# kaiidams/Kokoro-Align

Hardware: AMD Instinct MI355X
Metric: aligned audio-frames/sec (whole node), 50k x 5k lattice (higher is better)
Workload: dtype f32; 1 GPU; cfg2: T=50000 x V=64 log-probs, S=5000 phonemes (L=10001), beam_size=1000, max_move=4; batch of 8192 independent lattices per GPU per step, as 4 launches of 2048 on 4 streams; lattices_per_gpu=8192, parallelism=lattice-sharded x1, kernel_form=auto, backtrace=auto, streams_per_gpu=4

## Files before the change

### kokoro-align_amd/csrc/ka_device.hpp

```cpp
#pragma once
#include "ka_types.hpp"

namespace ka {

__device__ __forceinline__ float ninf() { return -__builtin_inff(); }

__device__ __forceinline__ float wave_ror1(float x)
{
    return __builtin_bit_cast(float, __builtin_amdgcn_mov_dpp(__builtin_bit_cast(int, x), 0x13C, 0xF, 0xF, false));
}
__device__ __forceinline__ uint32_t shl1_in(uint32_t w, uint64_t mask)
{
    uint32_t r;
    uint64_t carry_out;
    asm("v_addc_co_u32 %0, %1, %2, %2, %3" : "=v"(r), "=&s"(carry_out) : "v"(w), "s"(mask));
    return r;
}
__device__ __forceinline__ float select_by_mask(float a, float b, uint64_t mask)
{
    float r;
    asm("v_cndmask_b32 %0, %1, %2, %3" : "=v"(r) : "v"(a), "v"(b), "s"(mask));
    return r;
}
__device__ __forceinline__ float bperm(int byte_addr, float src)
{
    return __builtin_bit_cast(float, __builtin_amdgcn_ds_bpermute(byte_addr, __builtin_bit_cast(int, src)));
}
__device__ __forceinline__ float first_lane(float x)
{
    return __builtin_bit_cast(float, __builtin_amdgcn_readfirstlane(__builtin_bit_cast(int, x)));
}

__device__ __forceinline__ float row_load(uint32_t lane_byte_off, const void *row_base )
{
    float r;
    asm volatile("global_load_dword %0, %1, %2" : "=v"(r) : "v"(lane_byte_off), "s"(row_base) : "memory");
    return r;
}
__device__ __forceinline__ void row_reload(float &r, uint32_t lane_byte_off, const void *row_base )
{
    asm volatile("global_load_dword %0, %1, %2" : "+v"(r) : "v"(lane_byte_off), "s"(row_base) : "memory");
}
typedef uint32_t u32x4 __attribute__((ext_vector_type(4)));
__device__ __forceinline__ u32x4 lp_descriptor(const void *base, uint64_t bytes)
{
    const uint64_t a = reinterpret_cast<uint64_t>(base);
    const uint32_t n = bytes > 0xffffffffull ? 0xffffffffu : (uint32_t)bytes;
    return u32x4{(uint32_t)__builtin_amdgcn_readfirstlane((int)(uint32_t)a), (uint32_t)__builtin_amdgcn_readfirstlane((int)((uint32_t)(a >> 32) & 0xffffu)),
                 (uint32_t)__builtin_amdgcn_readfirstlane((int)n), 0x00020000u};
}
__device__ __forceinline__ void row_reload_buf(float &r, uint32_t lane_byte_off, u32x4 rsrc , uint32_t row_byte_off )
{
    asm volatile("buffer_load_dword %0, %1, %2, %3 offen" : "+v"(r) : "v"(lane_byte_off), "s"(rsrc), "s"(row_byte_off) : "memory");
}
template <int N>
__device__ __forceinline__ void row_wait(float &r)
{
    asm volatile("s_waitcnt vmcnt(%1)" : "+v"(r) : "i"(N) : "memory");
}

__device__ __forceinline__ void row_wait_n(float &r, int n)
{
    switch (n) {
    case 0: row_wait<0>(r); break;
    case 1: row_wait<1>(r); break;
    case 2: row_wait<2>(r); break;
    case 3: row_wait<3>(r); break;
    case 4: row_wait<4>(r); break;
    case 5: row_wait<5>(r); break;
    case 6: row_wait<6>(r); break;
    case 7: row_wait<7>(r); break;
    case 8: row_wait<8>(r); break;
    case 9: row_wait<9>(r); break;
    case 10: row_wait<10>(r); break;
    case 11: row_wait<11>(r); break;
    case 12: row_wait<12>(r); break;
    case 13: row_wait<13>(r); break;
    case 14: row_wait<14>(r); break;
    case 15: row_wait<15>(r); break;
    case 16: row_wait<16>(r); break;
    case 17: row_wait<17>(r); break;
    case 18: row_wait<18>(r); break;
    case 19: row_wait<19>(r); break;
    case 20: row_wait<20>(r); break;
    case 21: row_wait<21>(r); break;
    case 22: row_wait<22>(r); break;
    case 23: row_wait<23>(r); break;
    case 24: row_wait<24>(r); break;
    case 25: row_wait<25>(r); break;
    case 26: row_wait<26>(r); break;
    case 27: row_wait<27>(r); break;
    case 28: row_wait<28>(r); break;
    case 29: row_wait<29>(r); break;
    case 30: row_wait<30>(r); break;
    case 31: row_wait<31>(r); break;
    default: row_wait<0>(r); break;
    }
}

struct BandMasks {
    uint64_t m0, m1, m2, m3, m4, m5, m6, m7, m8, m9, m10, m11, m12, m13, m14, m15;
    template <int K>
    __device__ __forceinline__ uint64_t &at()
    {
        if constexpr (K == 0) return m0;
        else if constexpr (K == 1) return m1;
        else if constexpr (K == 2) return m2;
        else if constexpr (K == 3) return m3;
        else if constexpr (K == 4) return m4;
        else if constexpr (K == 5) return m5;
        else if constexpr (K == 6) return m6;
        else if constexpr (K == 7) return m7;
        else if constexpr (K == 8) return m8;
        else if constexpr (K == 9) return m9;
        else if constexpr (K == 10) return m10;
        else if constexpr (K == 11) return m11;
        else if constexpr (K == 12) return m12;
        else if constexpr (K == 13) return m13;
        else if constexpr (K == 14) return m14;
        else return m15;
    }
};
template <int K>
__device__ __forceinline__ void band_rebuild_one(BandMasks &mk, uint32_t lo, uint32_t hi)
{
    const uint32_t first = (lo + 15u - (uint32_t)K) >> 4;
    const uint32_t last = (hi + 15u - (uint32_t)K) >> 4;
    const uint32_t cnt = last - first;
    const uint64_t m = cnt >= 64u ? ~0ull : ((1ull << cnt) - 1ull);
    const uint32_t r = first & 63u;
    mk.at<K>() = r ? ((m << r) | (m >> (64u - r))) : m;
    if constexpr (K < 15) band_rebuild_one<K + 1>(mk, lo, hi);
}
__device__ __forceinline__ void band_rebuild(BandMasks &mk, uint32_t lo, uint32_t hi) { band_rebuild_one<0>(mk, lo, hi); }
__device__ __forceinline__ void band_toggle(BandMasks &mk, uint32_t p)
{
    const uint64_t bit = 1ull << ((p >> 4) & 63u);
    const uint32_t k = p & 15u;
    asm volatile(
        "s_bitcmp1_b32 %16, 3\n\t"
        "s_cbranch_scc1 .Lka_8_16_%=\n\t"
        "s_bitcmp1_b32 %16, 2\n\t"
        "s_cbranch_scc1 .Lka_4_8_%=\n\t"
        "s_bitcmp1_b32 %16, 1\n\t"
        "s_cbranch_scc1 .Lka_2_4_%=\n\t"
        "s_bitcmp1_b32 %16, 0\n\t"
        "s_cbranch_scc1 .Lka_1_2_%=\n\t"
        "s_xor_b64 %0, %0, %17\n\t"
        "s_branch .Lka_end_%=\n\t"
        ".Lka_1_2_%=:\n\t"
        "s_xor_b64 %1, %1, %17\n\t"
        "s_branch .Lka_end_%=\n\t"
        ".Lka_2_4_%=:\n\t"
        "s_bitcmp1_b32 %16, 0\n\t"
        "s_cbranch_scc1 .Lka_3_2_%=\n\t"
        "s_xor_b64 %2, %2, %17\n\t"
        "s_branch .Lka_end_%=\n\t"
        ".Lka_3_2_%=:\n\t"
        "s_xor_b64 %3, %3, %17\n\t"
        "s_branch .Lka_end_%=\n\t"
        ".Lka_4_8_%=:\n\t"
        "s_bitcmp1_b32 %16, 1\n\t"
        "s_cbranch_scc1 .Lka_6_4_%=\n\t"
        "s_bitcmp1_b32 %16, 0\n\t"
        "s_cbranch_scc1 .Lka_5_2_%=\n\t"
        "s_xor_b64 %4, %4, %17\n\t"
        "s_branch .Lka_end_%=\n\t"
        ".Lka_5_2_%=:\n\t"
        "s_xor_b64 %5, %5, %17\n\t"
        "s_branch .Lka_end_%=\n\t"
        ".Lka_6_4_%=:\n\t"
        "s_bitcmp1_b32 %16, 0\n\t"
        "s_cbranch_scc1 .Lka_7_2_%=\n\t"
        "s_xor_b64 %6, %6, %17\n\t"
        "s_branch .Lka_end_%=\n\t"
        ".Lka_7_2_%=:\n\t"
        "s_xor_b64 %7, %7, %17\n\t"
        "s_branch .Lka_end_%=\n\t"
        ".Lka_8_16_%=:\n\t"
        "s_bitcmp1_b32 %16, 2\n\t"
        "s_cbranch_scc1 .Lka_12_8_%=\n\t"
        "s_bitcmp1_b32 %16, 1\n\t"
        "s_cbranch_scc1 .Lka_10_4_%=\n\t"
        "s_bitcmp1_b32 %16, 0\n\t"
        "s_cbranch_scc1 .Lka_9_2_%=\n\t"
        "s_xor_b64 %8, %8, %17\n\t"
        "s_branch .Lka_end_%=\n\t"
        ".Lka_9_2_%=:\n\t"
        "s_xor_b64 %9, %9, %17\n\t"
        "s_branch .Lka_end_%=\n\t"
        ".Lka_10_4_%=:\n\t"
        "s_bitcmp1_b32 %16, 0\n\t"
        "s_cbranch_scc1 .Lka_11_2_%=\n\t"
        "s_xor_b64 %10, %10, %17\n\t"
        "s_branch .Lka_end_%=\n\t"
        ".Lka_11_2_%=:\n\t"
        "s_xor_b64 %11, %11, %17\n\t"
        "s_branch .Lka_end_%=\n\t"
        ".Lka_12_8_%=:\n\t"
        "s_bitcmp1_b32 %16, 1\n\t"
        "s_cbranch_scc1 .Lka_14_4_%=\n\t"
        "s_bitcmp1_b32 %16, 0\n\t"
        "s_cbranch_scc1 .Lka_13_2_%=\n\t"
        "s_xor_b64 %12, %12, %17\n\t"
        "s_branch .Lka_end_%=\n\t"
        ".Lka_13_2_%=:\n\t"
        "s_xor_b64 %13, %13, %17\n\t"
        "s_branch .Lka_end_%=\n\t"
        ".Lka_14_4_%=:\n\t"
        "s_bitcmp1_b32 %16, 0\n\t"
        "s_cbranch_scc1 .Lka_15_2_%=\n\t"
        "s_xor_b64 %14, %14, %17\n\t"
        "s_branch .Lka_end_%=\n\t"
        ".Lka_15_2_%=:\n\t"
        "s_xor_b64 %15, %15, %17\n\t"
        "s_branch .Lka_end_%=\n\t"
        ".Lka_end_%=:\n\t"
        : "+s"(mk.m0), "+s"(mk.m1), "+s"(mk.m2), "+s"(mk.m3), "+s"(mk.m4), "+s"(mk.m5), "+s"(mk.m6), "+s"(mk.m7),
          "+s"(mk.m8), "+s"(mk.m9), "+s"(mk.m10), "+s"(mk.m11), "+s"(mk.m12), "+s"(mk.m13), "+s"(mk.m14), "+s"(mk.m15)
        : "s"(k), "s"(bit)
        : "scc");
}
__device__ __forceinline__ uint32_t pair_mask(int n)
{
    n = n < 0 ? 0 : n;
    return n >= 16 ? 0x55555555u : (((1u << (2 * n)) - 1u) & 0x55555555u);
}
__device__ __forceinline__ uint32_t band_pairs(uint32_t lo, uint32_t hi, int blk)
{
    const int p0 = blk * 16;
    return pair_mask((int)hi - p0) & ~pair_mask((int)lo - p0);
}
__device__ __forceinline__ void load_block_labels(gci32_t labx, int blk, int (&la)[8])
{
    gci4_t p = (gci4_t)(labx + (size_t)blk * 8);
    const v4i_t a = p[0], b = p[1];
    la[0] = a.x; la[1] = a.y; la[2] = a.z; la[3] = a.w;
    la[4] = b.x; la[5] = b.y; la[6] = b.z; la[7] = b.w;
}

__device__ __forceinline__ uint64_t feq(float a, float b) { return __builtin_amdgcn_fcmpf(a, b, 1 ); }

template <int M>
__device__ __forceinline__ void cell_blank(float a0, float a1, float a3, float e, float &m, uint32_t &word)
{
    const float c0 = a0 + e;
    if constexpr (M == 1) {
        m = c0;
        word = (word << 2) | 3u;
    } else {
        const float c1 = a1 + e;
        if constexpr (M <= 3) {
            m = __builtin_fmaxf(c0, c1);
            word = (shl1_in(word, feq(c0, m)) << 1) | 1u;
        } else {
            const float c3 = a3 + e;
            m = __builtin_fmaxf(__builtin_fmaxf(c0, c1), c3);
            word = shl1_in(shl1_in(word, feq(c0, m)), feq(c1, m));
        }
    }
}
template <int M, bool ZL>
__device__ __forceinline__ void cell_label(float a0, float a1, float a2, float a3, float e, float veto,
                                           float &m, uint32_t &word)
{
    const float c0 = a0 + e;
    if constexpr (M == 1) {
        m = c0;
        word = (word << 2) | 3u;
    } else {
        const float c1 = a1 + e;
        if constexpr (M == 2) {
            m = __builtin_fmaxf(c0, c1);
            const uint64_t e0 = feq(c0, m);
            word = shl1_in((word << 1) | 1u, e0);
        } else {
            float c2 = a2 + e;
            if constexpr (ZL) c2 = __builtin_fminf(c2, veto);
            if constexpr (M == 3) {
                m = __builtin_fmaxf(__builtin_fmaxf(c0, c1), c2);
                const uint64_t e0 = feq(c0, m), e1 = feq(c1, m);
                word = shl1_in(shl1_in(word, e0 | e1), ~e1 | e0);
            } else {
                const float c3 = a3 + e;
                m = __builtin_fmaxf(__builtin_fmaxf(__builtin_fmaxf(c0, c1), c2), c3);
                const uint64_t e0 = feq(c0, m), e1 = feq(c1, m), e2 = feq(c2, m);
                word = shl1_in(shl1_in(word, e0 | e1), e0 | (e2 & ~e1));
            }
        }
    }
}
__device__ __forceinline__ uint32_t blank_to_uniform(uint32_t x)
{
    const uint32_t h = (x >> 1) & 0x11111111u, l = x & 0x11111111u;
    return (x & 0xCCCCCCCCu) | ((h | l) << 1) | h;
}
__device__ __forceinline__ int bp_decode(uint32_t code) { return (int)(3u & ~code); }
__device__ __forceinline__ uint32_t live_pairs(uint32_t live2, uint32_t word, uint32_t band2)
{
    const uint32_t stay = (word >> 1) & (word | 0x11111111u);
    return (live2 | ~stay) & band2;
}

template <int M>
__device__ __forceinline__ float cell_blank_max(float a0, float a1, float a3)
{
    if constexpr (M == 1) return a0;
    if constexpr (M <= 3) return __builtin_fmaxf(a0, a1);
    return __builtin_fmaxf(__builtin_fmaxf(a0, a1), a3);
}
template <int M, bool ZL>
__device__ __forceinline__ float cell_label_max(float a0, float a1, float a2, float a3, float veto)
{
    if constexpr (M == 1) return a0;
    if constexpr (M == 2) return __builtin_fmaxf(a0, a1);
    if constexpr (ZL) a2 = __builtin_fminf(a2, veto);
    if constexpr (M == 3) return __builtin_fmaxf(__builtin_fmaxf(a0, a1), a2);
    return __builtin_fmaxf(__builtin_fmaxf(__builtin_fmaxf(a0, a1), a2), a3);
}
template <int M, bool ZL>
__device__ __forceinline__ f32x2 label_pair_max(float l1, float b1, float l0, float b0, float p1, float p2, float veto1, float veto0)
{
    if constexpr (M == 4 && !ZL) {
        const float m0 = __builtin_fmaxf(l0, b0);
        return f32x2{__builtin_fmaxf(__builtin_fmaxf(m0, p1), p2), __builtin_fmaxf(__builtin_fmaxf(l1, b1), m0)};
    } else {
        return f32x2{cell_label_max<M, ZL>(l0, b0, p1, p2, veto0), cell_label_max<M, ZL>(l1, b1, l0, b0, veto1)};
    }
}
#define KA_P(P, k) (P)[2 * ((k) >> 2) + ((k) & 1)][((k) >> 1) & 1]
__device__ __forceinline__ float lds_col(const float *row, int byte_addr)
{
    return *reinterpret_cast<const float *>(reinterpret_cast<const char *>(row) + byte_addr);
}
template <int M, bool ZL, int G>
__device__ __forceinline__ void frame_scores(f32x2 (&P)[8], float h1, float h2, float h3, f32x2 (&E)[4], const float (&vz)[8],
                                             f32x2 e00, const int (&la)[8], const float *next_row)
{
    const float b0 = P[2 * G][0], l0 = P[2 * G + 1][0], b1 = P[2 * G][1], l1 = P[2 * G + 1][1];
    const float p1 = G > 0 ? P[2 * (G > 0 ? G - 1 : 0) + 1][1] : h1;
    const float p2 = G > 0 ? P[2 * (G > 0 ? G - 1 : 0)][1] : h2;
    const float p3 = G > 0 ? P[2 * (G > 0 ? G - 1 : 0) + 1][0] : h3;
    f32x2 ml, mb;
    ml = label_pair_max<M, ZL>(l1, b1, l0, b0, p1, p2, vz[2 * G + 1], vz[2 * G]);
    mb[1] = cell_blank_max<M>(b1, l0, p1);
    mb[0] = cell_blank_max<M>(b0, p1, p3);
    P[2 * G + 1] = ml + E[G];
    P[2 * G] = mb + e00;
    E[G][0] = lds_col(next_row, la[2 * G]);
    E[G][1] = lds_col(next_row, la[2 * G + 1]);
    if constexpr (G > 0) frame_scores<M, ZL, G - 1>(P, h1, h2, h3, E, vz, e00, la, next_row);
}

template <int K>
__device__ __forceinline__ void mask_scores(f32x2 (&P)[8], BandMasks &mk, float NINF)
{
    KA_P(P, K) = select_by_mask(NINF, KA_P(P, K), mk.at<K>());
    if constexpr (K > 0) mask_scores<K - 1>(P, mk, NINF);
}

template <int M, bool ZL, int K>
__device__ __forceinline__ void frame_cells(float (&sc)[16], float h1, float h2, float h3, float (&ec)[8],
                                            const float (&vz)[8], float e0, BandMasks &mk, float NINF, uint32_t &word,
                                            const int (&la)[8], float next_row)
{
    const float a0 = sc[K];
    const float a1 = K >= 1 ? sc[K >= 1 ? K - 1 : 0] : h1;
    const float a2 = K >= 2 ? sc[K >= 2 ? K - 2 : 0] : (K == 1 ? h1 : h2);
    const float a3 = K >= 3 ? sc[K >= 3 ? K - 3 : 0] : (K == 2 ? h1 : (K == 1 ? h2 : h3));
    float m;
    if constexpr (K & 1) {
        cell_label<M, ZL>(a0, a1, a2, a3, ec[K >> 1], vz[K >> 1], m, word);
        ec[K >> 1] = bperm(la[K >> 1], next_row);
    } else {
        cell_blank<M>(a0, a1, a3, e0, m, word);
    }
    sc[K] = select_by_mask(NINF, m, mk.at<K>());
    if constexpr (K % 4 == 0) __builtin_amdgcn_sched_barrier(0);
    if constexpr (K > 0) frame_cells<M, ZL, K - 1>(sc, h1, h2, h3, ec, vz, e0, mk, NINF, word, la, next_row);
}



__device__ __forceinline__ int lattice_of_chunk(const Lattice *__restrict__ lats, int n, int64_t g)
{
    int lo = 0, hi = n - 1;
    while (lo < hi) {
        const int mid = (lo + hi + 1) >> 1;
        if (lats[mid].chunk0 <= g) lo = mid; else hi = mid - 1;
    }
    return lo;
}
__device__ __forceinline__ int chunks_of(int T) { return (T - 1) / kCkFrames + 1; }

__device__ __forceinline__ float wave_shr1(float first, float x)
{
    return __builtin_bit_cast(float, __builtin_amdgcn_update_dpp(__builtin_bit_cast(int, first), __builtin_bit_cast(int, x), 0x138, 0xF, 0xF, false));
}

__device__ __forceinline__ uint32_t cu_slot()
{
    uint32_t hw, xcc;
    asm volatile("s_getreg_b32 %0, hwreg(HW_REG_HW_ID)" : "=s"(hw));
    asm volatile("s_getreg_b32 %0, hwreg(HW_REG_XCC_ID)" : "=s"(xcc));
    return ((xcc & 7u) << 8) | ((hw >> 8) & 0xffu);
}

}
```

### kokoro-align_amd/csrc/ka_wave_forward.hpp

```cpp
#pragma once
#include "ka_device.hpp"

namespace ka {

__global__ __launch_bounds__(256) void prep_labels_kernel(const Lattice *__restrict__ lats, int32_t *meta)
{
    const Lattice &d = lats[blockIdx.x];
    int bad = 0, zero = 0;
    for (int i = threadIdx.x; i < d.labx_len; i += blockDim.x) {
        int v = 0;
        if (i < d.S) {
            int l = d.labels[i];
            if (l < 0 || l >= d.V) { bad = 1; l = 0; }
            if (l == 0) zero = 1;
            v = l * 4;
        }
        d.labx[i] = v;
    }
    int32_t *m = meta_of(meta, d.idx);
    if (bad) atomicMin(&m[0], kStatusBadLabel);
    if (zero) atomicOr(&m[2], 1);
}

template <int M, bool ZL>
__device__ __forceinline__ void forward_w16(const Lattice &d, int32_t *meta)
{
    constexpr int D = kRowDepth;
    const int lane = threadIdx.x;
    const uint32_t T = (uint32_t)__builtin_amdgcn_readfirstlane(d.T);
    const uint32_t L = (uint32_t)__builtin_amdgcn_readfirstlane(d.L);
    const uint32_t B = (uint32_t)__builtin_amdgcn_readfirstlane(d.beam);
    const uint32_t halfB = B >> 1;
    const uint32_t dq = L / T, dr = L % T;
    const float NINF = ninf();

    float sc[16];
#pragma unroll
    for (int k = 0; k < 16; ++k) sc[k] = NINF;
    if (lane == 0) sc[0] = 0.0f;
    uint32_t pres2 = lane == 0 ? 1u : 0u;
    bool pend_reset = false;
    bool reset_lane = false;

    int blk = lane;
    uint32_t blo = 0;
    int la[8];
    float vz[8];
    gci32_t labx = (gci32_t)d.labx;
    load_block_labels(labx, blk, la);
#pragma unroll
    for (int i = 0; i < 8; ++i) vz[i] = (ZL && la[i] == 0) ? NINF : __builtin_inff();

    uint32_t q = 0, rem = 0;
    uint32_t lo = 0, hi = B < L ? B : L;
    BandMasks mk;
    band_rebuild(mk, lo, hi);
    uint32_t band2 = band_pairs(lo, hi, blk);

    const uint32_t lane_off = (lane < d.V ? (uint32_t)lane : 0u) * 4u;
    const char *lp = reinterpret_cast<const char *>(d.lp);
    const size_t ld = (size_t)d.ld * 4;
    float rows[D];
#pragma unroll
    for (int i = 0; i < D; ++i) {
        const uint32_t tt = (uint32_t)i < T ? (uint32_t)i : T - 1;
        rows[i] = row_load(lane_off, lp + (size_t)tt * ld);
    }
#pragma unroll
    for (int i = 0; i < D; ++i) row_wait<0>(rows[i]);
    float e[8], e0[2];
#pragma unroll
    for (int i = 0; i < 8; ++i) e[i] = bperm(la[i], rows[0]);
    e0[0] = first_lane(rows[0]);
    float absum = __builtin_fabsf(rows[0]);

    const uint32_t *bp = reinterpret_cast<const uint32_t *>(d.bp);
    const uint32_t lane_store_off = (uint32_t)lane * 16u;

    const char *row_ahead = lp + (size_t)(D < T ? D : T - 1) * ld;
    uint32_t step_thr = dq != 0 ? 0u : T;
    asm("" : "+s"(step_thr));
    for (uint32_t tb = 0; tb < T; tb += D) {
        uint32_t gw[4];
#pragma unroll
        for (int i = 0; i < 4; ++i) asm("" : "=v"(gw[i]));
#pragma unroll
        for (int dd = 0; dd < D; ++dd) {
            const uint32_t t = tb + dd;
            if (t < T) {
                float h1 = wave_ror1(sc[15]), h2 = wave_ror1(sc[14]), h3 = wave_ror1(sc[13]);
                if (__builtin_expect(pend_reset, 0)) {
                    asm volatile("" ::: "memory");
                    const bool left_reset = __builtin_amdgcn_update_dpp(0, (int)reset_lane, 0x13C, 0xF, 0xF, false) != 0;
                    const bool kill = reset_lane && left_reset;
                    h1 = kill ? NINF : h1;
                    h2 = kill ? NINF : h2;
                    h3 = kill ? NINF : h3;
#pragma unroll
                    for (int k = 0; k < 16; ++k) sc[k] = reset_lane ? NINF : sc[k];
                    pres2 = reset_lane ? 0u : pres2;
                    pend_reset = false;
                }
                bool moved = false;
                rem += dr;
                if (__builtin_expect(rem >= step_thr, 0)) {
                    asm volatile("" ::: "memory");
                    q += dq;
                    if (rem >= T) { rem -= T; ++q; }
                    if (t + 1 != T) {
                        moved = true;
                        const int32_t dlo = (int32_t)q - (int32_t)halfB;
                        const uint32_t nlo = (uint32_t)(dlo > 0 ? dlo : 0);
                        if ((nlo >> 4) != blo) {
                            blo = nlo >> 4;
                            const int nb = (int)blo + ((lane - (int)blo) & 63);
                            reset_lane = nb != blk;
                            if (nb != blk) {
                                blk = nb;
                                load_block_labels(labx, blk, la);
#pragma unroll
                                for (int i = 0; i < 8; ++i) asm volatile("" : "+v"(la[i]));
                            }
                            pend_reset = true;
                        }
                    }
                }
                if (dd < D - 1) row_wait<D - 1>(rows[(dd + 1) % D]); else row_wait<D - 2>(rows[(dd + 1) % D]);
                const float rn = rows[(dd + 1) % D];
                e0[(dd + 1) & 1] = first_lane(rn);
                absum += __builtin_fabsf(rn);
                uint32_t word = 0;
                frame_cells<M, ZL, 15>(sc, h1, h2, h3, e, vz, e0[dd & 1], mk, NINF, word, la, rn);
                gw[dd] = word;
                pres2 = live_pairs(pres2, word, band2);
                row_reload(rows[dd], lane_off, row_ahead);
                row_ahead += t + D + 1 < T ? ld : 0;
                if (moved) {
                    const int32_t dlo = (int32_t)q - (int32_t)halfB;
                    const uint32_t nlo = (uint32_t)(dlo > 0 ? dlo : 0);
                    const uint32_t nhi = (L - nlo < B) ? L : nlo + B;
                    if (nlo != lo || nhi != hi) {
                        if (nhi - hi <= 1u && nlo - lo <= 1u) {
                            if (nhi != hi) band_toggle(mk, hi);
                            if (nlo != lo) band_toggle(mk, lo);
                        } else {
                            band_rebuild(mk, nlo, nhi);
                        }
                        band2 = band_pairs(nlo, nhi, blk);
                        lo = nlo;
                        hi = nhi;
                        if (ZL && pend_reset) {
#pragma unroll
                            for (int i = 0; i < 8; ++i) vz[i] = la[i] == 0 ? NINF : __builtin_inff();
                        }
                    }
                }
            }
        }
        const u32x4 words = {gw[0], gw[1], gw[2], gw[3]};
        asm volatile("global_store_dwordx4 %0, %1, %2\n\ts_nop 1" : : "v"(lane_store_off), "v"(words), "s"(bp + (size_t)tb * 64) : "memory");
    }

#pragma unroll
    for (int i = 0; i < D; ++i) row_wait<0>(rows[i]);

    int32_t *m = meta_of(meta, d.idx);
    if (__builtin_amdgcn_ballot_w64((__builtin_bit_cast(uint32_t, absum) & 0x7fffffffu) > 0x7f800000u)) {
        if (lane == 0) {
            m[1] = -1;
            atomicMin(&m[0], kStatusNaN);
        }
        return;
    }
    int best = -1;
    if (pres2) best = blk * 16 + ((31 - __clz((int)pres2)) >> 1);
#pragma unroll
    for (int off = 32; off >= 1; off >>= 1) {
        const int o = __shfl_xor(best, off);
        best = o > best ? o : best;
    }
    if (best < 0) {
        if (lane == 0) {
            m[1] = -1;
            atomicMin(&m[0], kStatusEmptyBeam);
        }
    } else if ((best >> 4) == blk) {
        float v = sc[0];
#pragma unroll
        for (int k = 1; k < 16; ++k) v = (best & 15) == k ? sc[k] : v;
        m[1] = best;
        m[3] = __builtin_bit_cast(int32_t, v);
    }
}

template <int M, bool ZL>
__device__ __forceinline__ void forward_ck(const Lattice &d, int32_t *meta)
{
    constexpr int D = kRowDepth;
    const int lane = threadIdx.x;
    const uint32_t T = (uint32_t)__builtin_amdgcn_readfirstlane(d.T);
    const uint32_t L = (uint32_t)__builtin_amdgcn_readfirstlane(d.L);
    const uint32_t B = (uint32_t)__builtin_amdgcn_readfirstlane(d.beam);
    const uint32_t halfB = B >> 1;
    const uint32_t dq = L / T, dr = L % T;
    const float NINF = ninf();

    f32x2 P[8];
#pragma unroll
    for (int k = 0; k < 16; ++k) KA_P(P, k) = NINF;
    if (lane == 0) KA_P(P, 0) = 0.0f;
    float absum = 0.0f;

    int blk = lane;
    uint32_t blo = 0;
    int la[8];
    float vz[8];
    gci32_t labx = (gci32_t)d.labx;
    load_block_labels(labx, blk, la);
#pragma unroll
    for (int i = 0; i < 8; ++i) vz[i] = (ZL && la[i] == 0) ? NINF : __builtin_inff();

    uint32_t q = 0, rem = 0;
    uint32_t lo = 0, hi = B < L ? B : L;
    BandMasks mk;
    band_rebuild(mk, lo, hi);

    const uint32_t lane_off = (lane < d.V ? (uint32_t)lane : 0u) * 4u;
    const char *lp = reinterpret_cast<const char *>(d.lp);
    const size_t ld = (size_t)d.ld * 4;
    float rows[D];
#pragma unroll
    for (int i = 0; i < D; ++i) {
        const uint32_t tt = (uint32_t)i < T ? (uint32_t)i : T - 1;
        rows[i] = row_load(lane_off, lp + (size_t)tt * ld);
    }
#pragma unroll
    for (int i = 0; i < D; ++i) row_wait<0>(rows[i]);
    f32x2 E[4];
    float e0[2];
    __shared__ float lrow[64];
    lrow[lane] = rows[0];
#pragma unroll
    for (int i = 0; i < 8; ++i) E[i >> 1][i & 1] = lds_col(lrow, la[i]);
    e0[0] = first_lane(rows[0]);
    absum = __builtin_fabsf(rows[0]);

    const char *ckp = reinterpret_cast<const char *>(d.bp);
    const uint32_t ld32 = (uint32_t)__builtin_amdgcn_readfirstlane((int)(uint32_t)ld), last_row = (T - 1u) * ld32;
    uint32_t row_ahead = (D < T ? (uint32_t)D : T - 1u) * ld32;
    const u32x4 lp_rsrc = lp_descriptor(d.lp, (uint64_t)T * ld);
    const uint32_t thr_real = dq != 0 ? 0u : T;
    const uint32_t mask_every4 = 1024u - (B < L ? B : L) >= 8u * (M - 1) ? 0u : 4u;
    uint32_t thr = thr_real;
    asm("" : "+s"(thr));
    float h1 = wave_ror1(KA_P(P, 15)), h2 = wave_ror1(KA_P(P, 14)), h3 = wave_ror1(KA_P(P, 13));
    for (uint32_t tb = 0; tb < T; tb += D) {
#pragma unroll
        for (int dd = 0; dd < D; ++dd) {
            const uint32_t t = tb + dd;
            if (t < T) {
                row_wait<D - 2>(rows[(dd + 1) % D]);
                const float rn = rows[(dd + 1) % D];
                lrow[lane] = rn;
                e0[(dd + 1) & 1] = first_lane(rn);
                absum += __builtin_fabsf(rn);
                const float e0t = e0[dd & 1];
                frame_scores<M, ZL, 3>(P, h1, h2, h3, E, vz, f32x2{e0t, e0t}, la, lrow);
                row_reload_buf(rows[dd], lane_off, lp_rsrc, row_ahead);
                row_ahead = min(row_ahead + ld32, last_row);
                if (dd == D - 1 && ((tb | mask_every4) & 4u) != 0) {
                    mask_scores<15>(P, mk, NINF);
                    if (((tb + D) & (kCkFrames - 1)) == 0 && tb + D < T) {
                        const char *ck = ckp + ((size_t)((tb + D) / kCkFrames) - 1) * 4096;
#pragma unroll
                        for (int g = 0; g < 4; ++g) {
                            const f32x4 v = {KA_P(P, 4 * g), KA_P(P, 4 * g + 1), KA_P(P, 4 * g + 2), KA_P(P, 4 * g + 3)};
                            asm volatile("global_store_dwordx4 %0, %1, %2 offset:%3\n\ts_nop 1" : : "v"((uint32_t)lane * 64u), "v"(v), "s"(ck), "i"(16 * g) : "memory");
                        }
                    }
                }
                h1 = wave_ror1(KA_P(P, 15));
                h2 = wave_ror1(KA_P(P, 14));
                h3 = wave_ror1(KA_P(P, 13));
                rem += dr;
                if (__builtin_expect(rem >= thr, 0)) {
                    asm volatile("" ::: "memory");
                    thr = thr_real;
                    if (dd != D - 1 || ((tb | mask_every4) & 4u) == 0) {
                        mask_scores<15>(P, mk, NINF);
                        h1 = wave_ror1(KA_P(P, 15));
                        h2 = wave_ror1(KA_P(P, 14));
                        h3 = wave_ror1(KA_P(P, 13));
                    }
                    if (rem >= thr_real) {
                        q += dq;
                        if (rem >= T) { rem -= T; ++q; }
                        if (t + 1 != T) {
                            const int32_t dlo = (int32_t)q - (int32_t)halfB;
                            const uint32_t nlo = (uint32_t)(dlo > 0 ? dlo : 0);
                            const uint32_t nhi = (L - nlo < B) ? L : nlo + B;
                            if ((nlo >> 4) != blo) {
                                blo = nlo >> 4;
                                const int nb = (int)blo + ((lane - (int)blo) & 63);
                                const bool reset_lane = nb != blk;
                                if (reset_lane) {
                                    blk = nb;
                                    load_block_labels(labx, blk, la);
#pragma unroll
                                    for (int i = 0; i < 8; ++i) asm volatile("" : "+v"(la[i]));
                                }
                                const bool left_reset = __builtin_amdgcn_update_dpp(0, (int)reset_lane, 0x13C, 0xF, 0xF, false) != 0;
                                const bool kill = reset_lane && left_reset;
                                h1 = kill ? NINF : h1;
                                h2 = kill ? NINF : h2;
                                h3 = kill ? NINF : h3;
#pragma unroll
                                for (int k = 0; k < 16; ++k) KA_P(P, k) = reset_lane ? NINF : KA_P(P, k);
#pragma unroll
                                for (int i = 0; i < 8; ++i) E[i >> 1][i & 1] = lds_col(lrow, la[i]);
                                if constexpr (ZL) {
#pragma unroll
                                    for (int i = 0; i < 8; ++i) vz[i] = la[i] == 0 ? NINF : __builtin_inff();
                                }
                            }
                            if (nlo != lo || nhi != hi) {
                                if (nhi - hi <= 1u && nlo - lo <= 1u) {
                                    if (nhi != hi) band_toggle(mk, hi);
                                    if (nlo != lo) band_toggle(mk, lo);
                                } else {
                                    band_rebuild(mk, nlo, nhi);
                                }
                                lo = nlo;
                                hi = nhi;
                                thr = 0;
                            }
                        }
                    }
                }
            }
        }
    }
#pragma unroll
    for (int i = 0; i < D; ++i) row_wait<0>(rows[i]);

    int32_t *m = meta_of(meta, d.idx);
    mask_scores<15>(P, mk, NINF);
    const uint32_t abits = __builtin_bit_cast(uint32_t, absum) & 0x7fffffffu;
    if (__builtin_amdgcn_ballot_w64(abits > 0x7f800000u)) {
        if (lane == 0) {
            m[1] = -1;
            atomicMin(&m[0], kStatusNaN);
        }
        return;
    }
    if (__builtin_amdgcn_ballot_w64(abits >= __builtin_bit_cast(uint32_t, 1e30f))) {
        if (lane == 0) atomicOr(&m[2], kFlagExact);
        return;
    }
    float sc[16];
    uint32_t pres2 = 0;
#pragma unroll
    for (int k = 0; k < 16; ++k) {
        sc[k] = KA_P(P, k);
        pres2 |= sc[k] != NINF ? (1u << (2 * k)) : 0u;
    }
    int best = -1;
    if (pres2) best = blk * 16 + ((31 - __clz((int)pres2)) >> 1);
#pragma unroll
    for (int off = 32; off >= 1; off >>= 1) {
        const int o = __shfl_xor(best, off);
        best = o > best ? o : best;
    }
    if (best < 0) {
        if (lane == 0) {
            m[1] = -1;
            atomicMin(&m[0], kStatusEmptyBeam);
        }
    } else if ((best >> 4) == blk) {
        float v = sc[0];
#pragma unroll
        for (int k = 1; k < 16; ++k) v = (best & 15) == k ? sc[k] : v;
        m[1] = best;
        m[3] = __builtin_bit_cast(int32_t, v);
    }
}

constexpr int kFwdMinWaves = 4;
template <int M, bool ZL>
__global__ __launch_bounds__(64, kFwdMinWaves) void forward_w16_kernel(const Lattice *__restrict__ lats, int32_t *meta, int only_flagged)
{
    const Lattice &d = lats[blockIdx.x];
    const int flags = __builtin_amdgcn_readfirstlane(meta_of(meta, d.idx)[2]);
    if (((flags & kFlagZeroLabel) != 0) != ZL) return;
    if (only_flagged && !(flags & kFlagExact)) return;
    forward_w16<M, ZL>(d, meta);
}
template <int M, bool ZL>
__global__ __launch_bounds__(64, kFwdMinWaves) void forward_ck_kernel(const Lattice *__restrict__ lats, int32_t *meta)
{
    const Lattice &d = lats[blockIdx.x];
    const int flags = __builtin_amdgcn_readfirstlane(meta_of(meta, d.idx)[2]);
    if (((flags & kFlagZeroLabel) != 0) != ZL) return;
    if ((uint64_t)(uint32_t)d.T * (uint64_t)d.ld * 4ull > 0xffffffffull) {
        if (threadIdx.x == 0) atomicOr(&meta_of(meta, d.idx)[2], kFlagExact);
        return;
    }
    forward_ck<M, ZL>(d, meta);
}

__global__ __launch_bounds__(256) void forward_generic_kernel(const Lattice *__restrict__ lats, int32_t *meta)
{
    const Lattice &d = lats[blockIdx.x];
    const int tid = threadIdx.x;
    const int64_t T = d.T, L = d.L, B = d.beam;
    const int M = d.max_move;
    const int64_t W = d.W;
    float *scA = d.col, *scB = d.col + L;
    uint8_t *prA = reinterpret_cast<uint8_t *>(d.col + 2 * L), *prB = prA + L;
    uint8_t *bp = reinterpret_cast<uint8_t *>(d.bp);
    for (int64_t p = tid; p < L; p += 256) { prA[p] = 0; prB[p] = 0; }
    __syncthreads();
    if (tid == 0) { scA[0] = 0.0f; prA[0] = 1; }
    __syncthreads();
    int64_t plo = 0, phi = 1;
    for (int64_t t = 0; t < T; ++t) {
        int64_t lo = (L * t) / T - B / 2;
        lo = lo < 0 ? 0 : lo;
        const int64_t hi = (L - lo < B) ? L : lo + B;
        const float *row = d.lp + (size_t)t * (size_t)d.ld;
        for (int64_t p = lo + tid; p < hi; p += 256) {
            const int lab = (p & 1) ? (d.labx[p >> 1] >> 2) : 0;
            const float e = row[lab];
            float best = ninf();
            int bj = 0;
            for (int j = 0; j < M; ++j) {
                const int64_t u = p - j;
                if (u < 0) break;
                const bool pres = (u >= plo && u < phi) ? prA[u] != 0 : false;
                float c = pres ? scA[u] + e : ninf();
                if (j > 0 && (j & 1) == 0 && lab == 0) c = ninf();
                if (j == 0 || c > best) { best = c; bj = j; }
            }
            const int64_t ub = p - bj;
            prB[p] = (ub >= plo && ub < phi) ? prA[ub] : 0;
            scB[p] = best;
            bp[(size_t)t * (size_t)W + (size_t)(p - lo)] = (uint8_t)bj;
        }
        __syncthreads();
        { float *x = scA; scA = scB; scB = x; }
        { uint8_t *x = prA; prA = prB; prB = x; }
        plo = lo;
        phi = hi;
    }
    __shared__ int64_t s_best;
    if (tid == 0) s_best = -1;
    __syncthreads();
    int64_t mine = -1;
    for (int64_t p = plo + tid; p < phi; p += 256)
        if (prA[p]) mine = p;
    if (mine >= 0) atomicMax((long long *)&s_best, (long long)mine);
    __syncthreads();
    if (tid == 0) {
        int32_t *m = meta_of(meta, d.idx);
        if (s_best < 0) {
            m[1] = -1;
            atomicMin(&m[0], kStatusEmptyBeam);
        } else {
            m[1] = (int32_t)s_best;
            m[3] = __builtin_bit_cast(int32_t, scA[s_best]);
        }
    }
}

}
```

Before: 6.969 billion frames/s.

## Load log-prob rows in 4-row dwordx4 blocks staged through LDS double buffer

When the log-prob matrix is densely packed (ld=V=64, 16-byte aligned), the checkpointed forward kernel now fetches four consecutive frames per buffer_load_dwordx4 into a double-buffered LDS tile, rather than issuing one dword load per lane per frame. Emission heads are extracted with readlane. Separately, the band-mask cadence is generalised so masking can run less often when the band step pattern allows it. This cuts the number of memory instructions and waits per frame, at the cost of larger LDS use, a second template instantiation, and waits on a single outstanding load per 4 frames.

```diff
diff --git a/kokoro-align_amd/csrc/ka_device.hpp b/kokoro-align_amd/csrc/ka_device.hpp
--- a/kokoro-align_amd/csrc/ka_device.hpp
+++ b/kokoro-align_amd/csrc/ka_device.hpp
@@ -30,6 +30,10 @@
 {
     return __builtin_bit_cast(float, __builtin_amdgcn_readfirstlane(__builtin_bit_cast(int, x)));
 }
+__device__ __forceinline__ float lane_of(float x, int l)
+{
+    return __builtin_bit_cast(float, __builtin_amdgcn_readlane(__builtin_bit_cast(int, x), l));
+}
 
 __device__ __forceinline__ float row_load(uint32_t lane_byte_off, const void *row_base )
 {
@@ -52,6 +56,14 @@
 __device__ __forceinline__ void row_reload_buf(float &r, uint32_t lane_byte_off, u32x4 rsrc , uint32_t row_byte_off )
 {
     asm volatile("buffer_load_dword %0, %1, %2, %3 offen" : "+v"(r) : "v"(lane_byte_off), "s"(rsrc), "s"(row_byte_off) : "memory");
+}
+__device__ __forceinline__ void block_reload(f32x4 &r, uint32_t byte_off, u32x4 rsrc )
+{
+    asm volatile("buffer_load_dwordx4 %0, %1, %2, 0 offen" : "+v"(r) : "v"(byte_off), "s"(rsrc) : "memory");
+}
+__device__ __forceinline__ void block_wait(f32x4 &r)
+{
+    asm volatile("s_waitcnt vmcnt(0)" : "+v"(r) : : "memory");
 }
 template <int N>
 __device__ __forceinline__ void row_wait(float &r)
diff --git a/kokoro-align_amd/csrc/ka_wave_forward.hpp b/kokoro-align_amd/csrc/ka_wave_forward.hpp
--- a/kokoro-align_amd/csrc/ka_wave_forward.hpp
+++ b/kokoro-align_amd/csrc/ka_wave_forward.hpp
@@ -193,10 +193,11 @@
     }
 }
 
-template <int M, bool ZL>
-__device__ __forceinline__ void forward_ck(const Lattice &d, int32_t *meta)
+template <int M, bool ZL, bool BLK>
+__device__ __forceinline__ void forward_ck_body(const Lattice &d, int32_t *meta, float *lrow)
 {
     constexpr int D = kRowDepth;
+    constexpr int U = BLK ? 2 * D : D;
     const int lane = threadIdx.x;
     const uint32_t T = (uint32_t)__builtin_amdgcn_readfirstlane(d.T);
     const uint32_t L = (uint32_t)__builtin_amdgcn_readfirstlane(d.L);
@@ -228,47 +229,92 @@
     const uint32_t lane_off = (lane < d.V ? (uint32_t)lane : 0u) * 4u;
     const char *lp = reinterpret_cast<const char *>(d.lp);
     const size_t ld = (size_t)d.ld * 4;
-    float rows[D];
-#pragma unroll
-    for (int i = 0; i < D; ++i) {
-        const uint32_t tt = (uint32_t)i < T ? (uint32_t)i : T - 1;
-        rows[i] = row_load(lane_off, lp + (size_t)tt * ld);
-    }
-#pragma unroll
-    for (int i = 0; i < D; ++i) row_wait<0>(rows[i]);
+    const u32x4 lp_rsrc = lp_descriptor(d.lp, (uint64_t)T * ld);
+    [[maybe_unused]] float rows[D];
+    [[maybe_unused]] f32x4 rblk;
+    [[maybe_unused]] uint32_t blk_off = (uint32_t)lane * 16u;
     f32x2 E[4];
-    float e0[2];
-    __shared__ float lrow[64];
-    lrow[lane] = rows[0];
+    float e0[BLK ? 8 : 2];
+    if constexpr (BLK) {
+        asm("" : "=v"(rblk));
+        block_reload(rblk, blk_off, lp_rsrc);
+        block_wait(rblk);
+        *reinterpret_cast<f32x4 *>(lrow + lane * 4) = rblk;
+#pragma unroll
+        for (int r = 0; r < 4; ++r) e0[r] = lane_of(rblk[0], 16 * r);
+        absum = __builtin_fabsf(rblk[0]) + __builtin_fabsf(rblk[1]) + __builtin_fabsf(rblk[2]) + __builtin_fabsf(rblk[3]);
+        blk_off += 1024u;
+        __builtin_amdgcn_sched_barrier(0);
+        block_reload(rblk, blk_off, lp_rsrc);
+        __builtin_amdgcn_sched_barrier(0);
+        blk_off += 1024u;
+    } else {
+#pragma unroll
+        for (int i = 0; i < D; ++i) {
+            const uint32_t tt = (uint32_t)i < T ? (uint32_t)i : T - 1;
+            rows[i] = row_load(lane_off, lp + (size_t)tt * ld);
+        }
+#pragma unroll
+        for (int i = 0; i < D; ++i) row_wait<0>(rows[i]);
+        lrow[lane] = rows[0];
+        e0[0] = first_lane(rows[0]);
+        absum = __builtin_fabsf(rows[0]);
+    }
 #pragma unroll
     for (int i = 0; i < 8; ++i) E[i >> 1][i & 1] = lds_col(lrow, la[i]);
-    e0[0] = first_lane(rows[0]);
-    absum = __builtin_fabsf(rows[0]);
 
     const char *ckp = reinterpret_cast<const char *>(d.bp);
     const uint32_t ld32 = (uint32_t)__builtin_amdgcn_readfirstlane((int)(uint32_t)ld), last_row = (T - 1u) * ld32;
     uint32_t row_ahead = (D < T ? (uint32_t)D : T - 1u) * ld32;
-    const u32x4 lp_rsrc = lp_descriptor(d.lp, (uint64_t)T * ld);
     const uint32_t thr_real = dq != 0 ? 0u : T;
-    const uint32_t mask_every4 = 1024u - (B < L ? B : L) >= 8u * (M - 1) ? 0u : 4u;
+    const uint32_t P_static = 1024u - (B < L ? B : L) >= 8u * (M - 1) ? 8u : 4u;
+    const bool steps_mask = dq != 0 || (uint64_t)(P_static - 1u) * dr >= T;
+    const uint32_t mask_bits = steps_mask ? ((uint32_t)kCkFrames - 1u) & ~3u : (P_static - 1u) & ~3u;
     uint32_t thr = thr_real;
     asm("" : "+s"(thr));
     float h1 = wave_ror1(KA_P(P, 15)), h2 = wave_ror1(KA_P(P, 14)), h3 = wave_ror1(KA_P(P, 13));
-    for (uint32_t tb = 0; tb < T; tb += D) {
-#pragma unroll
-        for (int dd = 0; dd < D; ++dd) {
-            const uint32_t t = tb + dd;
+    for (uint32_t t0 = 0; t0 < T; t0 += U) {
+#pragma unroll
+        for (int u = 0; u < U; ++u) {
+            const int dd = u % D;
+            const uint32_t tb = t0 + (u - dd);
+            const uint32_t t = t0 + u;
             if (t < T) {
-                row_wait<D - 2>(rows[(dd + 1) % D]);
-                const float rn = rows[(dd + 1) % D];
-                lrow[lane] = rn;
-                e0[(dd + 1) & 1] = first_lane(rn);
-                absum += __builtin_fabsf(rn);
-                const float e0t = e0[dd & 1];
-                frame_scores<M, ZL, 3>(P, h1, h2, h3, E, vz, f32x2{e0t, e0t}, la, lrow);
-                row_reload_buf(rows[dd], lane_off, lp_rsrc, row_ahead);
-                row_ahead = min(row_ahead + ld32, last_row);
-                if (dd == D - 1 && ((tb | mask_every4) & 4u) != 0) {
+                const float *next_row = lrow;
+                float e0t;
+                if constexpr (BLK) {
+                    const int nu = (u + 1) % U;
+                    if (dd == D - 1) {
+                        block_wait(rblk);
+                        *reinterpret_cast<f32x4 *>(lrow + (nu / 4) * 256 + lane * 4) = rblk;
+#pragma unroll
+                        for (int r = 0; r < 4; ++r) e0[(nu / 4) * 4 + r] = lane_of(rblk[0], 16 * r);
+                        absum += __builtin_fabsf(rblk[0]);
+                        absum += __builtin_fabsf(rblk[1]);
+                        absum += __builtin_fabsf(rblk[2]);
+                        absum += __builtin_fabsf(rblk[3]);
+                        asm volatile("" : "+v"(absum));
+                        __builtin_amdgcn_sched_barrier(0);
+                        block_reload(rblk, blk_off, lp_rsrc);
+                        __builtin_amdgcn_sched_barrier(0);
+                        blk_off += 1024u;
+                    }
+                    next_row = lrow + (nu / 4) * 256 + (nu % 4) * 64;
+                    e0t = e0[u];
+                } else {
+                    row_wait<D - 2>(rows[(dd + 1) % D]);
+                    const float rn = rows[(dd + 1) % D];
+                    lrow[lane] = rn;
+                    e0[(dd + 1) & 1] = first_lane(rn);
+                    absum += __builtin_fabsf(rn);
+                    e0t = e0[dd & 1];
+                }
+                frame_scores<M, ZL, 3>(P, h1, h2, h3, E, vz, f32x2{e0t, e0t}, la, next_row);
+                if constexpr (!BLK) {
+                    row_reload_buf(rows[dd], lane_off, lp_rsrc, row_ahead);
+                    row_ahead = min(row_ahead + ld32, last_row);
+                }
+                if (dd == D - 1 && (~tb & mask_bits) == 0) {
                     mask_scores<15>(P, mk, NINF);
                     if (((tb + D) & (kCkFrames - 1)) == 0 && tb + D < T) {
                         const char *ck = ckp + ((size_t)((tb + D) / kCkFrames) - 1) * 4096;
@@ -286,7 +332,7 @@
                 if (__builtin_expect(rem >= thr, 0)) {
                     asm volatile("" ::: "memory");
                     thr = thr_real;
-                    if (dd != D - 1 || ((tb | mask_every4) & 4u) == 0) {
+                    if (dd != D - 1 || (~tb & mask_bits) != 0) {
                         mask_scores<15>(P, mk, NINF);
                         h1 = wave_ror1(KA_P(P, 15));
                         h2 = wave_ror1(KA_P(P, 14));
@@ -317,7 +363,7 @@
 #pragma unroll
                                 for (int k = 0; k < 16; ++k) KA_P(P, k) = reset_lane ? NINF : KA_P(P, k);
 #pragma unroll
-                                for (int i = 0; i < 8; ++i) E[i >> 1][i & 1] = lds_col(lrow, la[i]);
+                                for (int i = 0; i < 8; ++i) E[i >> 1][i & 1] = lds_col(next_row, la[i]);
                                 if constexpr (ZL) {
 #pragma unroll
                                     for (int i = 0; i < 8; ++i) vz[i] = la[i] == 0 ? NINF : __builtin_inff();
@@ -340,8 +386,12 @@
             }
         }
     }
-#pragma unroll
-    for (int i = 0; i < D; ++i) row_wait<0>(rows[i]);
+    if constexpr (BLK) {
+        block_wait(rblk);
+    } else {
+#pragma unroll
+        for (int i = 0; i < D; ++i) row_wait<0>(rows[i]);
+    }
 
     int32_t *m = meta_of(meta, d.idx);
     mask_scores<15>(P, mk, NINF);
@@ -383,6 +433,17 @@
         m[1] = best;
         m[3] = __builtin_bit_cast(int32_t, v);
     }
+}
+
+template <int M, bool ZL>
+__device__ __forceinline__ void forward_ck(const Lattice &d, int32_t *meta)
+{
+    __shared__ __attribute__((aligned(16))) float lrow[2 * 4 * 64];
+    const uint32_t base_lo = (uint32_t)__builtin_amdgcn_readfirstlane((int)(uint32_t)reinterpret_cast<uint64_t>(d.lp));
+    const bool blocks = __builtin_amdgcn_readfirstlane(d.ld) == 64 && __builtin_amdgcn_readfirstlane(d.V) == 64 && (base_lo & 15u) == 0 &&
+                        (uint32_t)__builtin_amdgcn_readfirstlane(d.T) <= (0xffffffffu - 4096u) / 256u;
+    if (blocks) forward_ck_body<M, ZL, true>(d, meta, lrow);
+    else forward_ck_body<M, ZL, false>(d, meta, lrow);
 }
 
 constexpr int kFwdMinWaves = 4;
```

Result: faster. 7.137 billion frames/s, median of 6 (+2.4%).
